# thu-ml/tianshou

Hardware: NVIDIA H100
Metric: transitions/sec through Algorithm.learn() (PPO, obs=17) (higher is better)
Workload: dtype f32 (MLP fwd/bwd, Adam), f64 (GAE scan, running return statistics)

## Files before the change

### include/ts_b200.h

```cpp
#ifndef TS_B200_H_
#define TS_B200_H_

#include <stddef.h>
#include <stdint.h>

#ifdef __cplusplus
extern "C" {
#endif

#define TS_B200_ABI_VERSION 1

typedef void* ts_stream_t;

enum { TS_F32 = 0, TS_F64 = 1 };

int ts_version(void);
const char* ts_last_error(void);
int64_t ts_launch_count(void);
void ts_reset_launch_count(void);

size_t ts_gae_workspace_bytes(int64_t n);
int ts_gae(const void* v_s, const void* v_s_next, int v_dtype, const double* rew,
           const uint8_t* terminated, const uint8_t* truncated, const uint8_t* extra_end,
           int terminated_ends, int64_t n, double gamma, double lam, double* rms_state,
// ... 47 lines not shown
                      ts_stream_t stream);
int ts_prio_update_weight(double* tree, int64_t bound, const int64_t* index, const void* td,
                          int td_dtype, int64_t n, double alpha, double eps, double* prio_minmax,
                          ts_stream_t stream);
int ts_prio_get_weight(const double* tree, int64_t bound, const int64_t* index, int64_t n,
                       const double* prio_minmax, double beta, int weight_norm, double* out,
                       ts_stream_t stream);

#define TS_AC_RELU 1
#define TS_AC_CATEGORICAL 2
typedef struct ts_actor_critic_desc {
    int32_t obs_dim;
    int32_t act_dim;
    int32_t hidden;
    int32_t flags;
    int64_t a_w1, a_b1, a_w2, a_b2, a_w3, a_b3, a_logstd;
    int64_t c_w1, c_b1, c_w2, c_b2, c_w3, c_b3;
    int64_t n_params;
} ts_actor_critic_desc;

int ts_critic_forward(const float* params, const ts_actor_critic_desc* desc ,
                      const float* obs0, float* v_out0, const float* obs1, float* v_out1,
                      int64_t n, ts_stream_t stream);
int ts_actor_logp(const float* params, const ts_actor_critic_desc* desc ,
                  const float* obs, const float* act, int64_t n, float* logp_out, float* mu_out,
                  ts_stream_t stream);

typedef struct ts_ppo_hparams {
    double eps_clip;
    double dual_clip;
    double vf_coef;
    double ent_coef;
    double max_grad_norm;
    double adv_eps;
    double lr, beta1, beta2, adam_eps, weight_decay;
    int32_t value_clip;
    int32_t advantage_normalization;
    int32_t loss_kind;
    int32_t optimizer;
} ts_ppo_hparams;
#define TS_LOSS_PPO 0
#define TS_LOSS_A2C 1
#define TS_OPT_ADAM 0
#define TS_OPT_RMSPROP 1

#define TS_PPO_STATS_STRIDE 8
// ... 7 lines not shown
                const float* logp_old, const float* v_s, const int32_t* perm, int64_t lo,
                int64_t hi, int64_t global_rows, const float* adv_moments, float* partials,
                int32_t* n_partials_out , ts_stream_t stream);
int ts_grad_reduce(const float* partials, int32_t n_partials, const ts_actor_critic_desc* desc,
                   float* grad, ts_stream_t stream);
int ts_minibatch_adv_sums(const float* adv, const int32_t* perm, int64_t lo, int64_t hi,
                          double* sums, ts_stream_t stream);
int ts_adv_moments_finalize(const double* sums, int64_t global_rows, float* out,
                            ts_stream_t stream);
int ts_clip_adam_step(float* params, float* grad, const float* partials, int32_t n_partials,
                      float* exp_avg, float* exp_avg_sq, int64_t* step_count,
                      const ts_actor_critic_desc* desc, const ts_ppo_hparams* hp, float* stats_row,
                      ts_stream_t stream);

int ts_ppo_update(float* params, float* grad, float* partials, float* exp_avg, float* exp_avg_sq,
                  int64_t* step_count, const ts_actor_critic_desc* desc, const ts_ppo_hparams* hp,
                  const float* obs, const float* obs_next, const float* act, const double* rew,
                  const uint8_t* terminated, const uint8_t* truncated, const uint8_t* extra_end,
                  float* v_s, float* returns, float* adv, const float* logp_old,
                  float* v_next_tmp, int64_t N, const int32_t* perm, int32_t repeat,
                  const int64_t* bounds , int32_t n_minibatch, int32_t recompute_adv,
                  double gamma, double lam, double* rms_state, double rms_eps, void* gae_ws,
                  void* adv_tmp, void* weight_image, float* stats, void* row_feed, ts_stream_t stream);

#define TS_PEER_HANDLE_BYTES 64
int ts_peer_alloc(int64_t bytes, void** ptr_out, uint8_t* handle_out );
int ts_peer_open(const uint8_t* handle, void** ptr_out);
int ts_peer_close(void* ptr);
int ts_peer_free(void* ptr);
int64_t ts_ppo_peer_buffer_bytes(const ts_actor_critic_desc* desc, int32_t world);

int ts_epoch_adv_sums(const float* adv, const int32_t* perm, int64_t lo0, int64_t mb_size, int64_t end,
                      int32_t n_minibatch, double* sums, ts_stream_t stream);
int ts_epoch_adv_finalize(const double* sums, int64_t lo0, int64_t mb_size, int64_t end, int32_t n_minibatch,
                          int32_t world, float* out, ts_stream_t stream);

int ts_ppo_epoch_multi(float* params, float* grad, float* partials, float* exp_avg, float* exp_avg_sq,
                       int64_t* step_count, const ts_actor_critic_desc* desc, const ts_ppo_hparams* hp,
                       const float* obs, const float* act, const float* adv, const float* returns,
                       const float* logp_old, const float* v_s, const int32_t* perm, int64_t lo0,
                       int64_t mb_size, int64_t end, int32_t n_minibatch, const float* adv_moments,
                       void* weight_image, float* stats, int32_t rank, int32_t world,
                       void* const* peer_buffers , ts_stream_t stream);

int ts_host_mt19937_permutation(uint32_t* key , int32_t* pos , int64_t n, int32_t* out);

// ... 139 lines not shown
```

### tianshou_b200/algorithm/modelfree/a2c.py

```python
from __future__ import annotations

import contextlib
import ctypes as C
import os
from abc import ABC
from dataclasses import dataclass
from typing import Any

import numpy as np
import torch

from ... import ops
from ..._cabi import GRAD_EXTRA, STATS_STRIDE, PPOHParams, load_library, to_device
from ...data import Batch, ReplayBuffer, SequenceSummaryStats
from ...parallel import world
from ...utils import RunningMeanStd
from ...utils.net.common import ActorCritic
from ..base import OnPolicyAlgorithm, TrainingStats
from ..flat_params import (
    DeviceScratch,
    FlatGroup,
    UnsupportedModelError,
    bind_optimizer,
    check_categorical_dist_fn,
    check_gaussian_dist_fn,
    optimizer_hyperparams,
)
# ... 15 lines not shown
def _upload(arr: np.ndarray, dev: torch.device, dtype: torch.dtype | None = None) -> torch.Tensor:
    t = to_device(arr, dev, non_blocking=True)
    if dtype is not None and t.dtype != dtype:
        t = t.to(dtype)
    return t


class ActorCriticOnPolicyAlgorithm(OnPolicyAlgorithm, ABC):

    minibatch_shuffle: str = "numpy"
    _shuffle_seed: int = 0
    _shuffle_epoch: int = 0

    def __init__(self, *, policy: ProbabilisticActorPolicy, critic: torch.nn.Module, optim: OptimizerFactory,
                 optim_include_actor: bool, max_grad_norm: float | None = None, gae_lambda: float = 0.95,
                 max_batchsize: int = 256, gamma: float = 0.99, return_scaling: bool = False,
                 rollout_partition: str = "per_rank", data_parallel: bool = True) -> None:
        super().__init__(policy=policy)
        if rollout_partition not in ("per_rank", "shared"):
            raise ValueError(f"rollout_partition must be 'per_rank' or 'shared', got {rollout_partition!r}")
        self.rollout_partition = rollout_partition
        self.data_parallel = bool(data_parallel)
        self._active_order: MinibatchOrder | None = None
        self.critic = critic
        assert 0.0 <= gae_lambda <= 1.0, f"GAE lambda should be in [0, 1] but got: {gae_lambda}"
        assert 0.0 <= gamma <= 1.0, f"discount factor gamma should be in [0, 1] but got: {gamma}"
        self.gae_lambda = gae_lambda
        self.max_batchsize = max_batchsize
        self._actor_critic = ActorCritic(self.policy.actor, self.critic)
        self._spec = parse_actor_critic(self.policy.actor, self.critic, split=not optim_include_actor)
        dev = next(self.policy.actor.parameters()).device
        if dev.type != "cuda":
            raise UnsupportedModelError(
                f"actor/critic live on {dev}; tianshou_b200 has no CPU path -- move them to a CUDA device first")
        if self._spec.categorical:
            check_categorical_dist_fn(self.policy.dist_fn, self._spec.act_dim, dev)
        else:
            check_gaussian_dist_fn(self.policy.dist_fn, self._spec.act_dim, dev)
        force_layered = os.environ.get("TS_B200_FORCE_LAYERED", "0") == "1"
        fused = fused_descriptor(self._spec) if optim_include_actor and not force_layered else None
        if fused is None:
            self._desc, self._layered = None, LayeredActorCritic(self._spec, dev)
            if self._ranks()[1] > 1:
                raise UnsupportedModelError("the layer-wise actor-critic path is single-GPU")
            self._flat = self._layered.critic_group
        else:
# ... 112 lines not shown
        batch.__dict__["info"] = Batch()
        batch.__dict__["policy"] = Batch()
        return batch, indices

    def _add_returns_and_advantages(self, batch: Batch, buffer: ReplayBuffer | None, indices: Any) -> Batch:
        self._flat.ensure_adopted()
        n = batch.obs.shape[0]
        v_s = self._buf("v_s", n, torch.float32)
        v_next = self._buf("v_next", n, torch.float32)
        r, w = self._ranks()
        if self._layered is not None:
            self._layered.critic_values(batch.obs, v_s)
            self._layered.critic_values(batch.obs_next, v_next)
        elif self.rollout_partition == "shared" and w > 1 and n % w == 0:
            import torch.distributed as dist
            lo, hi = r * (n // w), (r + 1) * (n // w)
            pair = self._buf("v_pair_local", (2, n // w), torch.float32)
            ops.critic_forward(self._flat.flat, self._desc, batch.obs[lo:hi], batch.obs_next[lo:hi], out=pair[0], out2=pair[1])
            full = self._buf("v_pair_full", (w, 2, n // w), torch.float32)
            dist.all_gather_into_tensor(full, pair)
            v_s.view(w, n // w).copy_(full[:, 0])
            v_next.view(w, n // w).copy_(full[:, 1])
        else:
            ops.critic_forward(self._flat.flat, self._desc, batch.obs, batch.obs_next, out=v_s, out2=v_next)
        rms = self._rms_device() if self.return_scaling else None
        adv = self._buf("adv", n, torch.float32)
        ret = self._buf("returns", n, torch.float32)
        moments = None
        if rms is not None and w > 1 and self.rollout_partition == "per_rank":
            moments = self._buf("rms_moments", 3, torch.float64)
        ops.gae(v_s, v_next, batch.rew, batch.terminated, batch.truncated, batch.get("_unfinished"),
                gamma=self.gamma, gae_lambda=self.gae_lambda, rms_state=rms, rms_eps=self._eps,
                out=(adv, ret), workspace=self._gae_workspace(n), batch_moments_out=moments)
        if moments is not None:
            self._merge_rms_across_ranks(rms, moments)
        batch.__dict__["v_s"], batch.__dict__["returns"], batch.__dict__["adv"] = v_s, ret, adv
        return batch

    def _gae_workspace(self, n: int) -> torch.Tensor:
        from ..._cabi import load_library
        need = int(load_library().ts_gae_workspace_bytes(n))
        return self._buf("gae_ws", max(need, 64), torch.uint8)

    def _rms_device(self) -> torch.Tensor:
        t = self._scratch.get("rms")
        if t is None:
            t = self._scratch["rms"] = self.ret_rms.device_state(self.device)
        return t

    def _rms_begin(self) -> None:
        if self.return_scaling:
            self._scratch["rms"] = self.ret_rms.device_state(self.device)

    def _rms_end(self) -> None:
        if self.return_scaling and "rms" in self._scratch:
            self.ret_rms.load_device_state(self._scratch.pop("rms"))

    def _merge_rms_across_ranks(self, rms: torch.Tensor, moments: torch.Tensor) -> None:
        from ...parallel import allgather_moments
        from ..._cabi import call, ptr, stream_ptr
        allm = allgather_moments(moments)
# ... 35 lines not shown
```

### tianshou_b200/algorithm/modelfree/ppo.py

```python
from __future__ import annotations

import ctypes as C
from typing import Any, Literal

import torch

from ... import ops
from ..._cabi import LOSS_A2C, call, ptr, stream_ptr
from ...data import Batch, ReplayBuffer
from ...data.batch import minibatch_bounds
from ...parallel import allreduce_sum_
from ..minibatch_order import shared_slice
from ..optim import OptimizerFactory
from .a2c import A2CTrainingStats, ActorCriticOnPolicyAlgorithm
from .reinforce import ProbabilisticActorPolicy


class FusedActorCriticUpdate(ActorCriticOnPolicyAlgorithm):

    recompute_adv: bool = False
    advantage_normalization: bool = False

    def _loss_hparams(self) -> Any:
        raise NotImplementedError
# ... 29 lines not shown
                        self._one_pass(batch, order.rows[r], bounds, hp, stats[r * n_mb:], r, rank, wsize)
            result = self._stats_from_device(stats)
        self._rms_end()
        self._flat.export_state(self.optim._optim)
        return result

    def _minibatch_adv_moments(self, batch: Batch, perm: torch.Tensor, lo: int, hi: int, world: int) -> torch.Tensor:
        st = stream_ptr(self.device)
        sums = self._buf("adv_sums", 2, torch.float64)
        call("ts_minibatch_adv_sums", ptr(batch.adv), ptr(perm), lo, hi, ptr(sums), st)
        if world > 1:
            allreduce_sum_(sums)
        adv_mom = self._buf("adv_mom", 2, torch.float32)
        call("ts_adv_moments_finalize", ptr(sums), (hi - lo) * world, ptr(adv_mom), st)
        return adv_mom

    def _device_passes(self, batch: Batch, perm_rows: torch.Tensor | None, bounds: list[tuple[int, int]], hp: Any,
                       stats: torch.Tensor, nrep: int, recompute: bool, feed: Any = None) -> None:
        f, dev = self._flat, self.device
        N, n_mb = batch.obs.shape[0], len(bounds)
        adv_tmp = self._buf("adv_tmp", 32 + 8 * n_mb, torch.uint8)
        adv_tmp.zero_()
        bounds_c = (C.c_int64 * (2 * n_mb))(*[x for b in bounds for x in b])
        call("ts_ppo_update", ptr(f.flat), ptr(f.grad), ptr(f.partials), ptr(f.exp_avg), ptr(f.exp_avg_sq), ptr(f.step_dev),
             C.byref(self._desc), C.byref(hp), ptr(batch.obs), ptr(batch.obs_next), ptr(batch.act),
             ptr(batch.rew), ptr(batch.terminated), ptr(batch.truncated), ptr(batch.get("_unfinished")),
             ptr(batch.v_s), ptr(batch.returns), ptr(batch.adv), ptr(batch.logp_old),
             ptr(self._buf("v_next", N, torch.float32)), N, ptr(perm_rows), nrep, bounds_c, n_mb,
             int(recompute), float(self.gamma), float(self.gae_lambda),
             ptr(self._rms_device()) if self.return_scaling else None, float(self._eps),
             ptr(self._gae_workspace(N)), ptr(adv_tmp), ptr(f.weight_image), ptr(stats), feed, stream_ptr(dev))

    def _peer_exchange(self, bounds: list[tuple[int, int]]):
        import os

        from ...parallel import PeerExchange
        if "peer_exchange" not in self._scratch:
            size = bounds[0][1] - bounds[0][0]
            regular = all(lo == bounds[0][0] + m * size and (m == len(bounds) - 1 or hi == lo + size)
                          for m, (lo, hi) in enumerate(bounds))
            usable = (os.environ.get("TS_B200_NO_P2P", "0") != "1" and regular
                      and self._flat.weight_image is not None and os.environ.get("TS_B200_FORCE_SIMT", "0") != "1")
            self._scratch["peer_exchange"] = PeerExchange.create(self._desc, self.device) if usable else None
        return self._scratch["peer_exchange"]

    def _fused_distributed_pass(self, batch: Batch, perm: torch.Tensor | None, bounds: list[tuple[int, int]], hp: Any,
                                stats: torch.Tensor, rank: int, wsize: int) -> None:
        f, st = self._flat, stream_ptr(self.device)
        ex = self._scratch["peer_exchange"]
        n_mb = len(bounds)
        lo0, size, end = bounds[0][0], bounds[0][1] - bounds[0][0], bounds[-1][1]
        adv_mom = None
        if self.advantage_normalization:
            sums = self._buf("epoch_adv_sums", 2 * n_mb, torch.float64)
# ... 120 lines not shown
```

### tianshou_b200/csrc/index.cu

```cuda
#include "common.cuh"

namespace {

using tsb::find_subbuffer;
using tsb::pymod;

struct BufMeta {
    const int64_t* offset;
    int64_t E;
    const uint8_t* done;
    const int64_t* last_index;
    const int64_t* lengths;
};

__device__ __forceinline__ int64_t next_one(const BufMeta& m, int64_t i) {
    const int64_t total = __ldg(m.offset + m.E);
    i = pymod(i, total);
    const int64_t e = find_subbuffer(m.offset, m.E, i);
    const int64_t start = __ldg(m.offset + e);
    int64_t len = __ldg(m.lengths + e);
    if (len < 1) len = 1;
    const int64_t last = __ldg(m.last_index + e);
    const int64_t end_flag = (m.done[i] != 0) | (i == last);
    return pymod(i - start + 1 - end_flag, len) + start;
// ... 181 lines not shown
    }
}
template <typename W>
__global__ void scatter_rows_kernel(const W* __restrict__ src, int64_t row_words,
                                    const int64_t* __restrict__ idx, int64_t n, W* __restrict__ dst) {
    const int64_t total = n * row_words;
    for (int64_t t = (int64_t)blockIdx.x * blockDim.x + threadIdx.x; t < total;
         t += (int64_t)gridDim.x * blockDim.x) {
        const int64_t p = t / row_words, w = t - p * row_words;
        dst[idx[p] * row_words + w] = src[t];
    }
}
__global__ void gather_bytes_kernel(const uint8_t* __restrict__ src, const int64_t* __restrict__ idx,
                                    int64_t n, uint8_t* __restrict__ dst) {
    const int64_t t = (int64_t)blockIdx.x * blockDim.x + threadIdx.x;
    if (t < n) dst[t] = src[idx[t]];
}

__global__ void narrow_kernel(const int64_t* __restrict__ src, int64_t n, int32_t* __restrict__ dst) {
    const int64_t t = (int64_t)blockIdx.x * blockDim.x + threadIdx.x;
    if (t < n) dst[t] = (int32_t)src[t];
}

inline unsigned blocks_for(int64_t n, int threads) { return (unsigned)((n + threads - 1) / threads); }

}

#define META_ARGS_OK(fn) \
    TS_REQUIRE(offset && done && last_index && lengths && E > 0, fn ": null buffer metadata")

extern "C" int ts_next_index(const int64_t* index, int64_t n, const int64_t* offset, int64_t E,
                             const uint8_t* done, const int64_t* last_index,
                             const int64_t* lengths, int64_t* out, ts_stream_t stream) {
    if (n == 0) return 0;
    META_ARGS_OK("ts_next_index");
    TS_REQUIRE(index && out, "ts_next_index: null index/out");
    BufMeta m{offset, E, done, last_index, lengths};
    step_index_kernel<true><<<blocks_for(n, 256), 256, 0, tsb::as_stream(stream)>>>(m, index, n, out);
    return tsb::check_launch("ts_next_index");
}

extern "C" int ts_prev_index(const int64_t* index, int64_t n, const int64_t* offset, int64_t E,
                             const uint8_t* done, const int64_t* last_index,
                             const int64_t* lengths, int64_t* out, ts_stream_t stream) {
    if (n == 0) return 0;
    META_ARGS_OK("ts_prev_index");
    TS_REQUIRE(index && out, "ts_prev_index: null index/out");
    BufMeta m{offset, E, done, last_index, lengths};
// ... 132 lines not shown
```

### tianshou_b200/csrc/mlp.cu

```cuda
#include <math.h>
#include <stdlib.h>

#include "common.cuh"
#include "optim_math.cuh"
#include "ppo_math.cuh"

namespace {

constexpr int H = 64;
constexpr int kRows = 128;
constexpr int kThreads = 256;
constexpr int LDH = H + 4;
constexpr int LDW3 = H + 4;
constexpr int LDO = 32;
constexpr int kMaxAct = 16;
constexpr int kMaxObs = 64;

struct NetOff {
    int w1t, b1, w2t, w2, b2, w3, b3, ls;
};
struct Layout {
    int KX, LDX, A;
    NetOff actor, critic;
    int X, H1, H2, ACT, DOUT, ROWV, RED;
// ... 648 lines not shown
int set_smem(K kernel, size_t bytes, const char* fn) {
    static thread_local size_t configured[tsb::kMaxDevices] = {};
    const int dev = tsb::device_ordinal();
    if (bytes > configured[dev]) {
        int optin = 0;
        TS_CUDA(cudaDeviceGetAttribute(&optin, cudaDevAttrMaxSharedMemoryPerBlockOptin, dev));
        TS_REQUIRE(bytes <= (size_t)optin, "%s: this network shape needs %zu bytes of shared memory per block, the device allows %d",
                   fn, bytes, optin);
        TS_CUDA(cudaFuncSetAttribute(kernel, cudaFuncAttributeMaxDynamicSharedMemorySize, (int)bytes));
        configured[dev] = bytes;
    }
    return 0;
}

}

namespace tsb {
bool tc_supported(const ts_actor_critic_desc& d);
int launch_ppo_grad_tc(const float* params, const ts_actor_critic_desc& d, const ts_ppo_hparams& hp, const float* obs,
                       const float* act, const float* adv, const float* ret, const float* logp_old, const float* v_s,
                       const int32_t* perm, int64_t lo, int64_t hi, int64_t global_rows, const float* adv_moments,
                       float* grad, cudaStream_t st);
int launch_forward_tc(int mode, const float* params, const ts_actor_critic_desc& d, const float* in0, float* out0,
                      const float* in1, float* out1, int64_t n, cudaStream_t st);
int launch_ppo_epoch_tc(float* params, const ts_actor_critic_desc& d, const ts_ppo_hparams& hp, const float* obs,
                        const float* act, const float* adv, const float* ret, const float* logp_old, const float* v_s,
                        const int32_t* perm, int64_t lo0, int64_t mb_size, int64_t end, int n_mb, const float* adv_moments,
                        float* partials, float* grad_scratch, float* exp_avg, float* exp_avg_sq, int64_t* step_count,
                        float* stats, void* weight_image, const PeerArgs& px, cudaStream_t st);
int64_t weight_image_bytes(const ts_actor_critic_desc& d);
static bool simt_forced() {
    static const bool f = [] { const char* e = getenv("TS_B200_FORCE_SIMT"); return e && e[0] == '1'; }();
    return f;
}
}

extern "C" int ts_critic_forward(const float* params, const ts_actor_critic_desc* desc,
                                 const float* obs0, float* v_out0, const float* obs1,
                                 float* v_out1, int64_t n, ts_stream_t stream) {
    if (check_desc(desc, "ts_critic_forward")) return 2;
    if (n == 0) return 0;
    TS_REQUIRE(params && obs0 && v_out0 && (!obs1 || v_out1), "ts_critic_forward: null pointer");
    if (tsb::tc_supported(*desc) && !tsb::simt_forced())
        return tsb::launch_forward_tc(0, params, *desc, obs0, v_out0, obs1, v_out1, n, tsb::as_stream(stream));
    const size_t smem = smem_bytes(*desc, 0);
    if (set_smem(critic_forward_kernel, smem, "ts_critic_forward")) return 1;
    const int64_t tiles = ((n + kRows - 1) / kRows) * (obs1 ? 2 : 1);
    const unsigned grid = (unsigned)tsb::imin((int64_t)tiles, tsb::num_sms());
    critic_forward_kernel<<<grid, kThreads, smem, tsb::as_stream(stream)>>>(params, *desc, obs0, v_out0, obs1, v_out1, n);
    return tsb::check_launch("ts_critic_forward");
}

extern "C" int ts_actor_logp(const float* params, const ts_actor_critic_desc* desc, const float* obs,
                             const float* act, int64_t n, float* logp_out, float* mu_out,
                             ts_stream_t stream) {
    if (check_desc(desc, "ts_actor_logp")) return 2;
    if (n == 0) return 0;
    TS_REQUIRE(params && obs && act && logp_out, "ts_actor_logp: null pointer");
    if (tsb::tc_supported(*desc) && !tsb::simt_forced())
        return tsb::launch_forward_tc(1, params, *desc, obs, logp_out, act, mu_out, n, tsb::as_stream(stream));
    const size_t smem = smem_bytes(*desc, 1);
    if (set_smem(actor_logp_kernel, smem, "ts_actor_logp")) return 1;
    const int64_t tiles = (n + kRows - 1) / kRows;
    const unsigned grid = (unsigned)tsb::imin((int64_t)tiles, tsb::num_sms());
    actor_logp_kernel<<<grid, kThreads, smem, tsb::as_stream(stream)>>>(params, *desc, obs, act, n, logp_out, mu_out);
    return tsb::check_launch("ts_actor_logp");
}

extern "C" int ts_ppo_grad(const float* params, const ts_actor_critic_desc* desc,
                           const ts_ppo_hparams* hp, const float* obs, const float* act,
                           const float* adv, const float* ret, const float* logp_old,
                           const float* v_s, const int32_t* perm, int64_t lo, int64_t hi,
                           int64_t global_rows, const float* adv_moments, float* partials,
                           int32_t* n_partials_out, ts_stream_t stream) {
    if (check_desc(desc, "ts_ppo_grad")) return 2;
    TS_REQUIRE(hp != nullptr, "ts_ppo_grad: null hparams");
    TS_REQUIRE(hi >= lo && global_rows > 0, "ts_ppo_grad: bad row range");
    if (n_partials_out) *n_partials_out = 0;
    if (hi == lo) return 0;
    TS_REQUIRE(params && obs && act && adv && ret && logp_old && v_s && partials && n_partials_out, "ts_ppo_grad: null pointer");
    {
        const int64_t tiles_ = (hi - lo + kRows - 1) / kRows;
        *n_partials_out = (int32_t)tsb::imin(tiles_, tsb::num_sms());
// ... 61 lines not shown
extern "C" int ts_make_permutation(uint64_t seed, int32_t first_epoch, int32_t n_epochs, int64_t n,
                                   int32_t* out, ts_stream_t stream) {
    if (n == 0 || n_epochs == 0) return 0;
    TS_REQUIRE(out && n > 0 && n < (1ll << 31) && n_epochs > 0, "ts_make_permutation: bad arguments");
    int bits = 1;
    while ((1ll << bits) < n) ++bits;
    const int half = (bits + 1) / 2 < 1 ? 1 : (bits + 1) / 2;
    const int64_t total = n * n_epochs;
    const unsigned grid = (unsigned)tsb::imin((int64_t)(total + 255) / 256, (int64_t)tsb::num_sms() * 8);
    permutation_kernel<<<grid, 256, 0, tsb::as_stream(stream)>>>(seed, first_epoch, n_epochs, n, half, out);
    return tsb::check_launch("ts_make_permutation");
}

extern "C" int ts_ppo_update(float* params, float* grad, float* partials, float* exp_avg, float* exp_avg_sq,
                             int64_t* step_count, const ts_actor_critic_desc* desc,
                             const ts_ppo_hparams* hp, const float* obs, const float* obs_next,
                             const float* act, const double* rew, const uint8_t* terminated,
                             const uint8_t* truncated, const uint8_t* extra_end, float* v_s,
                             float* returns, float* adv, const float* logp_old, float* v_next_tmp,
                             int64_t N, const int32_t* perm, int32_t repeat, const int64_t* bounds,
                             int32_t n_minibatch, int32_t recompute_adv, double gamma, double lam,
                             double* rms_state, double rms_eps, void* gae_ws, void* adv_tmp,
                             void* weight_image, float* stats, void* row_feed, ts_stream_t stream) {
    if (check_desc(desc, "ts_ppo_update")) return 2;
    TS_REQUIRE(hp && bounds && stats && partials && grad && repeat >= 0 && n_minibatch >= 0, "ts_ppo_update: bad arguments");
    TS_REQUIRE(!hp->advantage_normalization || adv_tmp, "ts_ppo_update: adv_tmp required");
    static const bool no_fuse = [] { const char* e = getenv("TS_B200_NO_FUSED_STEP"); return e && e[0] == '1'; }();
    const bool fused = tsb::tc_supported(*desc) && !tsb::simt_forced() && !no_fuse;
    double* adv_sums = static_cast<double*>(adv_tmp);
    float* adv_mom = adv_tmp ? reinterpret_cast<float*>(adv_sums + 2) : nullptr;
    float* epoch_mom = adv_tmp ? reinterpret_cast<float*>(static_cast<uint8_t*>(adv_tmp) + 32) : nullptr;
    bool regular = n_minibatch > 0;
    const int64_t lo0 = n_minibatch > 0 ? bounds[0] : 0, mb_size = n_minibatch > 0 ? bounds[1] - bounds[0] : 0;
    for (int m = 0; m < n_minibatch && regular; ++m) {
        regular = bounds[2 * m] == lo0 + (int64_t)m * mb_size && bounds[2 * m + 1] > bounds[2 * m] &&
                  (m == n_minibatch - 1 || bounds[2 * m + 1] == lo0 + (int64_t)(m + 1) * mb_size);
    }
    for (int r = 0; r < repeat; ++r) {
        if (recompute_adv && r > 0) {
            TS_REQUIRE(obs_next && rew && v_next_tmp && gae_ws, "ts_ppo_update: recompute needs obs_next/rew/scratch");
            if (int e = ts_critic_forward(params, desc, obs, v_s, obs_next, v_next_tmp, N, stream)) return e;
            if (int e = ts_gae(v_s, v_next_tmp, TS_F32, rew, terminated, truncated, extra_end, 1, N, gamma,
                               lam, rms_state, rms_eps, nullptr, adv, returns, TS_F32, gae_ws, stream)) return e;
        }
        const int32_t* pr = perm ? perm + (int64_t)r * N : nullptr;
        float* rows = stats + (int64_t)r * n_minibatch * TS_PPO_STATS_STRIDE;
        if (row_feed) {
            if (int e = ts_host_perm_feed_wait_row(row_feed, r, stream)) return e;
        }
        if (fused && regular) {
            const int64_t end = bounds[2 * n_minibatch - 1];
            if (hp->advantage_normalization) {
                epoch_adv_moments_kernel<<<n_minibatch, 1024, 0, tsb::as_stream(stream)>>>(adv, pr, lo0, mb_size, end, n_minibatch, epoch_mom);
                if (int e = tsb::check_launch("ts_ppo_update(adv moments)")) return e;
            }
            if (int e = tsb::launch_ppo_epoch_tc(params, *desc, *hp, obs, act, adv, returns, logp_old, v_s, pr, lo0, mb_size, end,
                                                 n_minibatch, hp->advantage_normalization ? epoch_mom : nullptr, partials, grad,
                                                 exp_avg, exp_avg_sq, step_count, rows, weight_image, tsb::PeerArgs{}, tsb::as_stream(stream))) return e;
            continue;
        }
        for (int m = 0; m < n_minibatch; ++m) {
            const int64_t lo = bounds[2 * m], hi = bounds[2 * m + 1];
            if (hp->advantage_normalization) {
                if (int e = ts_minibatch_adv_sums(adv, pr, lo, hi, adv_sums, stream)) return e;
// ... 60 lines not shown
```

### tianshou_b200/csrc/mlp_tc.cu

```cuda
#include <cuda_bf16.h>
#include <math.h>

#include <type_traits>

#include "common.cuh"
#include "optim_math.cuh"
#include "ppo_math.cuh"
#include "wgmma.cuh"

namespace {

constexpr int H = 64;
constexpr int kRows = 128;
constexpr int kThreads = 512;
constexpr int kCols = 16;
constexpr int kMaxAct = 16;
constexpr int NO = 16;

#ifdef TS_B200_DIAGNOSTICS
__device__ unsigned long long g_tc_timeline[32];
__device__ int g_tc_timeline_on = 0;
__device__ int g_tc_timeline_gate = 1;
__device__ __forceinline__ void tstamp(int slot) {
    if (g_tc_timeline_on && (int)blockIdx.x == g_tc_timeline_on - 1 && threadIdx.x == 0 && g_tc_timeline_gate) {
// ... 855 lines not shown
    SmemF s{};
    s.KXP = kxp;
    uint32_t o = 0;
    auto mat = [&](Mat& m, int rows, int cols) {
        m.base = sbase + o; m.part = mat_bytes(rows, cols); m.RS = (uint32_t)(cols / 8) * 128u; o += 3u * m.part;
    };
    mat(s.X, kRows, s.KXP);
    mat(s.H1, kRows, H);
    mat(s.W1, H, s.KXP);
    mat(s.W2, H, H);
    s.w3f = o;  o += kMaxAct * H * 4;
    s.b1 = o;   o += H * 4;
    s.b2 = o;   o += H * 4;
    s.b3 = o;   o += kMaxAct * 4;
    s.ls = o;   o += kMaxAct * 4;
    s.part = o; o += 2 * kRows * kMaxAct * 4;
    s.total = o;
    return s;
}

template <int MODE, int KXP>
__global__ void __launch_bounds__(kThreads, 1) forward_tc_kernel(
    const float* __restrict__ params, const ts_actor_critic_desc d, const float* __restrict__ in0,
    float* __restrict__ out0, const float* __restrict__ in1, float* __restrict__ out1, int64_t n) {
    extern __shared__ __align__(1024) uint8_t sm[];
    const int tid = threadIdx.x, lane = tid & 31;
    const uint32_t sbase = wg::smem_u32(sm);
    uint8_t* sm0 = sm - sbase;
    const SmemF S = make_smem_f(KXP, sbase);
    const int out_dim = MODE == 0 ? 1 : d.act_dim;
    const NetG g = MODE == 0 ? NetG{d.c_w1, d.c_b1, d.c_w2, d.c_b2, d.c_w3, d.c_b3, -1}
                             : NetG{d.a_w1, d.a_b1, d.a_w2, d.a_b2, d.a_w3, d.a_b3, d.a_logstd};
    stage_chunks(sm0, S.W1, H, d.obs_dim, S.KXP, [&](int o) { return params + g.w1 + (int64_t)o * d.obs_dim; });
    stage_chunks(sm0, S.W2, H, H, H, [&](int o) { return params + g.w2 + (int64_t)o * H; });
    float* w3f = reinterpret_cast<float*>(sm + S.w3f);
    float* b1 = reinterpret_cast<float*>(sm + S.b1);
    float* b2 = reinterpret_cast<float*>(sm + S.b2);
    float* b3 = reinterpret_cast<float*>(sm + S.b3);
    float* ls = reinterpret_cast<float*>(sm + S.ls);
    float* part = reinterpret_cast<float*>(sm + S.part);
    for (int e = tid; e < kMaxAct * H; e += kThreads) w3f[e] = (e >> 6) < out_dim ? __ldg(params + g.w3 + e) : 0.0f;
    for (int e = tid; e < H; e += kThreads) { b1[e] = __ldg(params + g.b1 + e); b2[e] = __ldg(params + g.b2 + e); }
    if (tid < kMaxAct) {
        b3[tid] = tid < out_dim ? __ldg(params + g.b3 + tid) : 0.0f;
        ls[tid] = (MODE == 1 && tid < out_dim) ? expf(__ldg(params + g.ls + tid)) : 1.0f;
    }

    const int64_t tiles_per = (n + kRows - 1) / kRows;
    const int64_t tiles = tiles_per * ((MODE == 0 && in1) ? 2 : 1);
    const int64_t my_n = tiles > (int64_t)blockIdx.x ? (tiles - blockIdx.x + gridDim.x - 1) / gridDim.x : 0;
    auto tile_of = [&](int64_t k) { return (int64_t)blockIdx.x + k * gridDim.x; };
    auto tile_src = [&](int64_t t, const float*& src, int64_t& row0, int& nrows, bool& second) {
        second = t >= tiles_per;
        row0 = (second ? t - tiles_per : t) * kRows;
        nrows = (int)tsb::imin((int64_t)kRows, n - row0);
        src = (MODE == 0 && second) ? in1 : in0;
    };
    auto x_load = [&](int64_t k, float (&xv)[8]) {
        const float* src; int64_t row0; int nrows; bool second;
        tile_src(tile_of(k), src, row0, nrows, second);
        chunk_load(kRows, d.obs_dim, S.KXP, [&](int r) {
            return r < nrows ? src + (row0 + r) * d.obs_dim : (const float*)nullptr;
        }, xv);
    };
    const int half = tid >> 8;
    const int r0 = lay_row0() + wg::frag_row(0);

    float xv[8];
    if (my_n > 0) x_load(0, xv);
    for (int64_t k = 0; k < my_n; ++k) {
        const float* src; int64_t row0; int nrows; bool second;
        tile_src(tile_of(k), src, row0, nrows, second);
        __syncthreads();
        chunk_store(sm0, S.X, kRows, S.KXP, xv);
        if (k + 1 < my_n) x_load(k + 1, xv);
        publish();
        float acc[kCols], h[kCols];
        if (S.KXP == 16) wg_gemm<2 * kCols, 1, 0, 0>(acc, S.X, lay_row0(), S.W1, lay_col0());
        else wg_gemm<2 * kCols, 2, 0, 0>(acc, S.X, lay_row0(), S.W1, lay_col0());
        epi_tanh(sm0, S.H1, acc, b1);
        publish();
        wg_gemm<2 * kCols, H / 16, 0, 0>(acc, S.H1, lay_row0(), S.W2, lay_col0());
#pragma unroll
        for (int e = 0; e < kCols; ++e) h[e] = tanh_mufu(acc[e] + b2[lay_col0() + wg::frag_col(e)]);
        for (int a = 0; a < out_dim; ++a) {
            float p0 = 0.0f, p1 = 0.0f;
#pragma unroll
            for (int i = 0; i < kCols / 4; ++i) {
                const float2 w = *reinterpret_cast<const float2*>(w3f + a * H + lay_col0() + wg::frag_col(4 * i));
                p0 = fmaf(h[4 * i], w.x, p0); p0 = fmaf(h[4 * i + 1], w.y, p0);
                p1 = fmaf(h[4 * i + 2], w.x, p1); p1 = fmaf(h[4 * i + 3], w.y, p1);
            }
            p0 += __shfl_xor_sync(0xffffffffu, p0, 1); p0 += __shfl_xor_sync(0xffffffffu, p0, 2);
            p1 += __shfl_xor_sync(0xffffffffu, p1, 1); p1 += __shfl_xor_sync(0xffffffffu, p1, 2);
            if ((lane & 3) == 0) {
                part[(half * kMaxAct + a) * kRows + r0] = p0;
                part[(half * kMaxAct + a) * kRows + r0 + 8] = p1;
            }
        }
        __syncthreads();
        if (tid < nrows) {
            const int r = tid;
            if (MODE == 0) {
                (second ? out1 : out0)[row0 + r] = (part[r] + part[kMaxAct * kRows + r]) + b3[0];
            } else {
                float lp = 0.0f;
                for (int a = 0; a < out_dim; ++a) {
                    const float mu = (part[a * kRows + r] + part[(kMaxAct + a) * kRows + r]) + b3[a];
                    lp += ppo::normal_logp_term(__ldg(in1 + (row0 + r) * out_dim + a), mu, ls[a]);
                    if (out1) out1[(row0 + r) * out_dim + a] = mu;
                }
                out0[row0 + r] = lp;
            }
        }
    }
}

}

#ifdef TS_B200_DIAGNOSTICS
extern "C" int ts_tc_timeline(int32_t enable, uint64_t* out32 ) {
    int on = enable;
    TS_CUDA(cudaMemcpyToSymbol(g_tc_timeline_on, &on, sizeof(int)));
    if (out32) TS_CUDA(cudaMemcpyFromSymbol(out32, g_tc_timeline, 32 * sizeof(unsigned long long)));
    return 0;
}
#endif
// ... 54 lines not shown
        cfg.gridDim = dim3(grid); cfg.blockDim = dim3(kThreads); cfg.dynamicSmemBytes = S.total; cfg.stream = st;
        cudaLaunchAttribute attr[1];
        attr[0].id = cudaLaunchAttributeCooperative;
        attr[0].val.cooperative = 1;
        cfg.attrs = attr; cfg.numAttrs = 1;
        const int64_t zero = 0;
        uint8_t* wimg = weight_image ? static_cast<uint8_t*>(weight_image) + kCtlBytes : nullptr;
        if (wimg) {
            TS_CUDA(cudaMemsetAsync(wimg, 0, 2 * (size_t)S.wblk_bytes, st));
            weight_image_build_kernel<KXP><<<(unsigned)((d.n_params + 255) / 256), 256, 0, st>>>(params, d, wimg);
            if (int e = check_launch("ts_ppo_update(weight image)")) return e;
        }
        TS_CUDA(cudaLaunchKernelEx(&cfg, ppo_tc_kernel<true, KXP>, (const float*)params, d, hp, obs, act, adv, ret, logp_old, v_s,
                                   perm, lo0, mb_size, end, n_mb, zero, adv_moments, partials, opt, wimg, px));
        return check_launch("ts_ppo_epoch(tc)");
    });
}

int64_t weight_image_bytes(const ts_actor_critic_desc& d) {
    return tc_supported(d) ? (int64_t)kCtlBytes + 2 * (int64_t)make_smem(kxp_of(d.obs_dim), 0).wblk_bytes : 0;
}

int launch_forward_tc(int mode, const float* params, const ts_actor_critic_desc& d, const float* in0, float* out0,
                      const float* in1, float* out1, int64_t n, cudaStream_t st) {
    return with_kxp(d.obs_dim, [&](auto kxp) {
        constexpr int KXP = decltype(kxp)::value;
        constexpr size_t smem = make_smem_f(KXP, 0).total;
        const int64_t tiles = ((n + kRows - 1) / kRows) * ((mode == 0 && in1) ? 2 : 1);
        const unsigned grid = (unsigned)imin(tiles, num_sms());
        if (mode == 0) {
            if (int e = opt_in_smem<forward_tc_kernel<0, KXP>>(smem)) return e;
            forward_tc_kernel<0, KXP><<<grid, kThreads, smem, st>>>(params, d, in0, out0, in1, out1, n);
        } else {
            if (int e = opt_in_smem<forward_tc_kernel<1, KXP>>(smem)) return e;
            forward_tc_kernel<1, KXP><<<grid, kThreads, smem, st>>>(params, d, in0, out0, in1, out1, n);
        }
        return check_launch(mode == 0 ? "ts_critic_forward(tc)" : "ts_actor_logp(tc)");
    });
}
}
```

### tianshou_b200/ops.py

```python
from __future__ import annotations

import ctypes as C
from dataclasses import dataclass

import numpy as np
import torch

from . import _cabi
from ._cabi import TS_F32, TS_F64, ActorCriticDesc, PPOHParams, call, ptr, stream_ptr, to_device


def _dev(device: torch.device | str | None) -> torch.device:
    _cabi.require_cuda()
    if device is None:
        return torch.device("cuda", torch.cuda.current_device())
    d = torch.device(device)
    if d.type != "cuda":
        raise _cabi.ExtensionMissingError(f"tianshou_b200 kernels need a CUDA device, got {d}")
    return d


def _dt(t: torch.dtype) -> int:
    if t == torch.float32:
        return TS_F32
# ... 213 lines not shown
         stream_ptr(tree.device))
    return out


def segtree_sample(tree: torch.Tensor, bound: int, u: torch.Tensor) -> torch.Tensor:
    out = torch.empty(u.numel(), dtype=torch.int64, device=tree.device)
    call("ts_segtree_sample", ptr(tree), bound, ptr(u), u.numel(), ptr(out), stream_ptr(tree.device))
    return out


def critic_forward(params: torch.Tensor, desc: ActorCriticDesc, obs: torch.Tensor,
                   obs2: torch.Tensor | None = None,
                   out: torch.Tensor | None = None, out2: torch.Tensor | None = None):
    n = obs.shape[0]
    if out is None:
        out = torch.empty(n, dtype=torch.float32, device=obs.device)
    if obs2 is not None and out2 is None:
        out2 = torch.empty(n, dtype=torch.float32, device=obs.device)
    call("ts_critic_forward", ptr(params), C.byref(desc), ptr(obs), ptr(out), ptr(obs2), ptr(out2), n,
         stream_ptr(obs.device))
    return (out, out2) if obs2 is not None else out


def actor_logp(params: torch.Tensor, desc: ActorCriticDesc, obs: torch.Tensor, act: torch.Tensor,
               want_mu: bool = False, out: torch.Tensor | None = None):
    n = obs.shape[0]
    if out is None:
        out = torch.empty(n, dtype=torch.float32, device=obs.device)
    mu = torch.empty((n, desc.act_dim), dtype=torch.float32, device=obs.device) if want_mu else None
    call("ts_actor_logp", ptr(params), C.byref(desc), ptr(obs), ptr(act), n, ptr(out), ptr(mu),
         stream_ptr(obs.device))
    return (out, mu) if want_mu else out


def make_permutation(seed: int, first_epoch: int, n_epochs: int, n: int, device: torch.device) -> torch.Tensor:
    out = torch.empty((n_epochs, n), dtype=torch.int32, device=device)
    call("ts_make_permutation", C.c_uint64(seed & (2**64 - 1)), int(first_epoch), int(n_epochs), int(n),
         ptr(out), stream_ptr(device))
    return out


def narrow_i64_i32(src: torch.Tensor) -> torch.Tensor:
    out = torch.empty(src.shape, dtype=torch.int32, device=src.device)
    call("ts_narrow_i64_i32", ptr(src), src.numel(), ptr(out), stream_ptr(src.device))
    return out

# ... 3 lines not shown
```

Before: 26.71 million.

## Deduplicate critic forward on obs_next rows that alias the following obs row

Adds a mark/compact kernel pair that detects rows where obs_next[i] is bitwise equal to obs[i+1] and builds a compacted list of the non-aliased rows. The tensor-core critic forward then evaluates only obs plus those extra rows and scatters V(obs[i+1]) into v_next[i], roughly halving critic forward work for contiguous rollouts. The map is built once per batch and reused when the PPO update recomputes advantages across repeats. In exchange it adds two small kernels, indexed gathers and scatters, and a device-side row count that the kernel must read.

Measured after the change: 28.07 million (median of 6 runs). 5.1% higher.

```diff
diff --git a/include/ts_b200.h b/include/ts_b200.h
--- a/include/ts_b200.h
+++ b/include/ts_b200.h
@@ -93,6 +93,12 @@
 int ts_critic_forward(const float* params, const ts_actor_critic_desc* desc ,
                       const float* obs0, float* v_out0, const float* obs1, float* v_out1,
                       int64_t n, ts_stream_t stream);
+int64_t ts_next_alias_workspace_bytes(int64_t n);
+int ts_next_alias_map(const float* obs, const float* obs_next, int64_t n, int32_t obs_dim, uint8_t* alias,
+                      int32_t* extra, int32_t* n_extra, void* workspace, ts_stream_t stream);
+int ts_critic_forward_dedup(const float* params, const ts_actor_critic_desc* desc , const float* obs,
+                            const float* obs_next, const uint8_t* alias, const int32_t* extra,
+                            const int32_t* n_extra, float* v_s, float* v_next, int64_t n, ts_stream_t stream);
 int ts_actor_logp(const float* params, const ts_actor_critic_desc* desc ,
                   const float* obs, const float* act, int64_t n, float* logp_out, float* mu_out,
                   ts_stream_t stream);
@@ -146,6 +152,17 @@
                   const int64_t* bounds , int32_t n_minibatch, int32_t recompute_adv,
                   double gamma, double lam, double* rms_state, double rms_eps, void* gae_ws,
                   void* adv_tmp, void* weight_image, float* stats, void* row_feed, ts_stream_t stream);
+int ts_ppo_update_dedup(float* params, float* grad, float* partials, float* exp_avg, float* exp_avg_sq,
+                        int64_t* step_count, const ts_actor_critic_desc* desc, const ts_ppo_hparams* hp,
+                        const float* obs, const float* obs_next, const float* act, const double* rew,
+                        const uint8_t* terminated, const uint8_t* truncated, const uint8_t* extra_end,
+                        float* v_s, float* returns, float* adv, const float* logp_old,
+                        float* v_next_tmp, int64_t N, const int32_t* perm, int32_t repeat,
+                        const int64_t* bounds , int32_t n_minibatch, int32_t recompute_adv,
+                        double gamma, double lam, double* rms_state, double rms_eps, void* gae_ws,
+                        void* adv_tmp, void* weight_image, float* stats, void* row_feed,
+                        const uint8_t* next_alias, const int32_t* next_extra, const int32_t* n_next_extra,
+                        ts_stream_t stream);
 
 #define TS_PEER_HANDLE_BYTES 64
 int ts_peer_alloc(int64_t bytes, void** ptr_out, uint8_t* handle_out );
diff --git a/tianshou_b200/algorithm/modelfree/a2c.py b/tianshou_b200/algorithm/modelfree/a2c.py
--- a/tianshou_b200/algorithm/modelfree/a2c.py
+++ b/tianshou_b200/algorithm/modelfree/a2c.py
@@ -3,6 +3,7 @@
 import contextlib
 import ctypes as C
 import os
+import weakref
 from abc import ABC
 from dataclasses import dataclass
 from typing import Any
@@ -64,6 +65,7 @@
         self.rollout_partition = rollout_partition
         self.data_parallel = bool(data_parallel)
         self._active_order: MinibatchOrder | None = None
+        self._next_alias: tuple[Any, Any, ops.NextAliasMap] | None = None
         self.critic = critic
         assert 0.0 <= gae_lambda <= 1.0, f"GAE lambda should be in [0, 1] but got: {gae_lambda}"
         assert 0.0 <= gamma <= 1.0, f"discount factor gamma should be in [0, 1] but got: {gamma}"
@@ -222,7 +224,11 @@
             v_s.view(w, n // w).copy_(full[:, 0])
             v_next.view(w, n // w).copy_(full[:, 1])
         else:
-            ops.critic_forward(self._flat.flat, self._desc, batch.obs, batch.obs_next, out=v_s, out2=v_next)
+            amap = self._next_alias_map(batch, build=buffer is not None)
+            if amap is not None:
+                ops.critic_forward_dedup(self._flat.flat, self._desc, batch.obs, batch.obs_next, amap, out=v_s, out2=v_next)
+            else:
+                ops.critic_forward(self._flat.flat, self._desc, batch.obs, batch.obs_next, out=v_s, out2=v_next)
         rms = self._rms_device() if self.return_scaling else None
         adv = self._buf("adv", n, torch.float32)
         ret = self._buf("returns", n, torch.float32)
@@ -237,6 +243,20 @@
         batch.__dict__["v_s"], batch.__dict__["returns"], batch.__dict__["adv"] = v_s, ret, adv
         return batch
 
+    def _next_alias_map(self, batch: Batch, build: bool = False) -> ops.NextAliasMap | None:
+        obs, obs_next = batch.obs, batch.obs_next
+        if build:
+            n = obs.shape[0]
+            amap = ops.NextAliasMap(self._buf("next_alias", n, torch.uint8), self._buf("next_extra", n, torch.int32),
+                                    self._buf("next_extra_count", 1, torch.int32))
+            need = int(load_library().ts_next_alias_workspace_bytes(n))
+            ops.next_alias_map(obs, obs_next, out=amap, workspace=self._buf("next_alias_ws", max(need, 4), torch.uint8))
+            self._next_alias = (weakref.ref(obs), weakref.ref(obs_next), amap)
+        if self._next_alias is None:
+            return None
+        ref_obs, ref_next, amap = self._next_alias
+        return amap if ref_obs() is obs and ref_next() is obs_next else None
+
     def _gae_workspace(self, n: int) -> torch.Tensor:
         from ..._cabi import load_library
         need = int(load_library().ts_gae_workspace_bytes(n))
diff --git a/tianshou_b200/algorithm/modelfree/ppo.py b/tianshou_b200/algorithm/modelfree/ppo.py
--- a/tianshou_b200/algorithm/modelfree/ppo.py
+++ b/tianshou_b200/algorithm/modelfree/ppo.py
@@ -75,14 +75,16 @@
         adv_tmp = self._buf("adv_tmp", 32 + 8 * n_mb, torch.uint8)
         adv_tmp.zero_()
         bounds_c = (C.c_int64 * (2 * n_mb))(*[x for b in bounds for x in b])
-        call("ts_ppo_update", ptr(f.flat), ptr(f.grad), ptr(f.partials), ptr(f.exp_avg), ptr(f.exp_avg_sq), ptr(f.step_dev),
+        amap = self._next_alias_map(batch) if recompute else None
+        call("ts_ppo_update_dedup", ptr(f.flat), ptr(f.grad), ptr(f.partials), ptr(f.exp_avg), ptr(f.exp_avg_sq), ptr(f.step_dev),
              C.byref(self._desc), C.byref(hp), ptr(batch.obs), ptr(batch.obs_next), ptr(batch.act),
              ptr(batch.rew), ptr(batch.terminated), ptr(batch.truncated), ptr(batch.get("_unfinished")),
              ptr(batch.v_s), ptr(batch.returns), ptr(batch.adv), ptr(batch.logp_old),
              ptr(self._buf("v_next", N, torch.float32)), N, ptr(perm_rows), nrep, bounds_c, n_mb,
              int(recompute), float(self.gamma), float(self.gae_lambda),
              ptr(self._rms_device()) if self.return_scaling else None, float(self._eps),
-             ptr(self._gae_workspace(N)), ptr(adv_tmp), ptr(f.weight_image), ptr(stats), feed, stream_ptr(dev))
+             ptr(self._gae_workspace(N)), ptr(adv_tmp), ptr(f.weight_image), ptr(stats), feed,
+             *((ptr(amap.alias), ptr(amap.extra), ptr(amap.count)) if amap is not None else (None, None, None)), stream_ptr(dev))
 
     def _peer_exchange(self, bounds: list[tuple[int, int]]):
         import os
diff --git a/tianshou_b200/csrc/index.cu b/tianshou_b200/csrc/index.cu
--- a/tianshou_b200/csrc/index.cu
+++ b/tianshou_b200/csrc/index.cu
@@ -227,8 +227,87 @@
     if (t < n) dst[t] = (int32_t)src[t];
 }
 
+constexpr int kAliasThreads = 256;
+
+__global__ void __launch_bounds__(kAliasThreads) next_alias_mark_kernel(
+    const uint32_t* __restrict__ obs, const uint32_t* __restrict__ obs_next, int64_t n, int width,
+    uint8_t* __restrict__ alias, int32_t* __restrict__ block_extra) {
+    const int lane = threadIdx.x & 31;
+    const int64_t i0 = (int64_t)blockIdx.x * kAliasThreads + (threadIdx.x & ~31);
+    const int64_t rows = tsb::imin(32, n - 1 - i0);
+    const uint32_t* a = obs_next + i0 * width;
+    const uint32_t* b = obs + (i0 + 1) * width;
+    unsigned differs = 0u;
+    for (int64_t w = lane; w < rows * width; w += 32) {
+        if (a[w] != b[w]) differs |= 1u << (unsigned)(w / width);
+    }
+    differs = __reduce_or_sync(0xffffffffu, differs);
+    const int64_t i = i0 + lane;
+    const bool same = lane < rows && !((differs >> lane) & 1u);
+    if (i < n) alias[i] = same ? 1 : 0;
+    const int cnt = __syncthreads_count(i < n && !same);
+    if (threadIdx.x == 0) block_extra[blockIdx.x] = cnt;
+}
+
+__global__ void __launch_bounds__(kAliasThreads) next_alias_compact_kernel(
+    const uint8_t* __restrict__ alias, int64_t n, const int32_t* __restrict__ block_extra,
+    int32_t* __restrict__ extra, int32_t* __restrict__ n_extra) {
+    __shared__ int s_warp[kAliasThreads / 32];
+    __shared__ int s_base;
+    const int tid = threadIdx.x, lane = tid & 31, warp = tid >> 5;
+    int before_blocks = 0;
+    for (int b = tid; b < (int)blockIdx.x; b += kAliasThreads) before_blocks += block_extra[b];
+#pragma unroll
+    for (int off = 16; off > 0; off >>= 1) before_blocks += __shfl_xor_sync(0xffffffffu, before_blocks, off);
+    if (lane == 0) s_warp[warp] = before_blocks;
+    __syncthreads();
+    if (tid == 0) {
+        int base = 0;
+        for (int w = 0; w < kAliasThreads / 32; ++w) base += s_warp[w];
+        s_base = base;
+    }
+    __syncthreads();
+    const int64_t i = (int64_t)blockIdx.x * kAliasThreads + tid;
+    const bool keep = i < n && alias[i] == 0;
+    const unsigned bal = __ballot_sync(0xffffffffu, keep);
+    const int base = s_base;
+    __syncthreads();
+    if (lane == 0) s_warp[warp] = __popc(bal);
+    __syncthreads();
+    int before = 0, total = 0;
+    for (int w = 0; w < kAliasThreads / 32; ++w) {
+        if (w < warp) before += s_warp[w];
+        total += s_warp[w];
+    }
+    if (keep) extra[base + before + __popc(bal & ((1u << lane) - 1u))] = (int32_t)i;
+    if (blockIdx.x == gridDim.x - 1 && tid == 0) *n_extra = base + total;
+}
+
 inline unsigned blocks_for(int64_t n, int threads) { return (unsigned)((n + threads - 1) / threads); }
 
+}
+
+extern "C" int64_t ts_next_alias_workspace_bytes(int64_t n) {
+    return n > 0 ? 4 * (int64_t)blocks_for(n, kAliasThreads) : 0;
+}
+
+extern "C" int ts_next_alias_map(const float* obs, const float* obs_next, int64_t n, int32_t obs_dim, uint8_t* alias,
+                                 int32_t* extra, int32_t* n_extra, void* workspace, ts_stream_t stream) {
+    TS_REQUIRE(n >= 0 && n < (1ll << 31) && obs_dim >= 1, "ts_next_alias_map: bad shape");
+    TS_REQUIRE(n_extra, "ts_next_alias_map: null n_extra");
+    cudaStream_t st = tsb::as_stream(stream);
+    if (n == 0) {
+        TS_CUDA(cudaMemsetAsync(n_extra, 0, sizeof(int32_t), st));
+        return 0;
+    }
+    TS_REQUIRE(obs && obs_next && alias && extra && workspace, "ts_next_alias_map: null pointer");
+    int32_t* block_extra = static_cast<int32_t*>(workspace);
+    const unsigned grid = blocks_for(n, kAliasThreads);
+    next_alias_mark_kernel<<<grid, kAliasThreads, 0, st>>>(reinterpret_cast<const uint32_t*>(obs),
+                                                           reinterpret_cast<const uint32_t*>(obs_next), n, obs_dim, alias, block_extra);
+    if (tsb::check_launch("ts_next_alias_map/mark")) return 1;
+    next_alias_compact_kernel<<<grid, kAliasThreads, 0, st>>>(alias, n, block_extra, extra, n_extra);
+    return tsb::check_launch("ts_next_alias_map");
 }
 
 #define META_ARGS_OK(fn) \
diff --git a/tianshou_b200/csrc/mlp.cu b/tianshou_b200/csrc/mlp.cu
--- a/tianshou_b200/csrc/mlp.cu
+++ b/tianshou_b200/csrc/mlp.cu
@@ -694,7 +694,8 @@
                        const int32_t* perm, int64_t lo, int64_t hi, int64_t global_rows, const float* adv_moments,
                        float* grad, cudaStream_t st);
 int launch_forward_tc(int mode, const float* params, const ts_actor_critic_desc& d, const float* in0, float* out0,
-                      const float* in1, float* out1, int64_t n, cudaStream_t st);
+                      const float* in1, float* out1, int64_t n, const uint8_t* alias, const int32_t* extra,
+                      const int32_t* n_extra, cudaStream_t st);
 int launch_ppo_epoch_tc(float* params, const ts_actor_critic_desc& d, const ts_ppo_hparams& hp, const float* obs,
                         const float* act, const float* adv, const float* ret, const float* logp_old, const float* v_s,
                         const int32_t* perm, int64_t lo0, int64_t mb_size, int64_t end, int n_mb, const float* adv_moments,
@@ -714,13 +715,24 @@
     if (n == 0) return 0;
     TS_REQUIRE(params && obs0 && v_out0 && (!obs1 || v_out1), "ts_critic_forward: null pointer");
     if (tsb::tc_supported(*desc) && !tsb::simt_forced())
-        return tsb::launch_forward_tc(0, params, *desc, obs0, v_out0, obs1, v_out1, n, tsb::as_stream(stream));
+        return tsb::launch_forward_tc(0, params, *desc, obs0, v_out0, obs1, v_out1, n, nullptr, nullptr, nullptr, tsb::as_stream(stream));
     const size_t smem = smem_bytes(*desc, 0);
     if (set_smem(critic_forward_kernel, smem, "ts_critic_forward")) return 1;
     const int64_t tiles = ((n + kRows - 1) / kRows) * (obs1 ? 2 : 1);
     const unsigned grid = (unsigned)tsb::imin((int64_t)tiles, tsb::num_sms());
     critic_forward_kernel<<<grid, kThreads, smem, tsb::as_stream(stream)>>>(params, *desc, obs0, v_out0, obs1, v_out1, n);
     return tsb::check_launch("ts_critic_forward");
+}
+
+extern "C" int ts_critic_forward_dedup(const float* params, const ts_actor_critic_desc* desc, const float* obs,
+                                       const float* obs_next, const uint8_t* alias, const int32_t* extra,
+                                       const int32_t* n_extra, float* v_s, float* v_next, int64_t n, ts_stream_t stream) {
+    if (check_desc(desc, "ts_critic_forward_dedup")) return 2;
+    if (n == 0) return 0;
+    TS_REQUIRE(params && obs && obs_next && alias && extra && n_extra && v_s && v_next, "ts_critic_forward_dedup: null pointer");
+    if (tsb::tc_supported(*desc) && !tsb::simt_forced())
+        return tsb::launch_forward_tc(0, params, *desc, obs, v_s, obs_next, v_next, n, alias, extra, n_extra, tsb::as_stream(stream));
+    return ts_critic_forward(params, desc, obs, v_s, obs_next, v_next, n, stream);
 }
 
 extern "C" int ts_actor_logp(const float* params, const ts_actor_critic_desc* desc, const float* obs,
@@ -730,7 +742,7 @@
     if (n == 0) return 0;
     TS_REQUIRE(params && obs && act && logp_out, "ts_actor_logp: null pointer");
     if (tsb::tc_supported(*desc) && !tsb::simt_forced())
-        return tsb::launch_forward_tc(1, params, *desc, obs, logp_out, act, mu_out, n, tsb::as_stream(stream));
+        return tsb::launch_forward_tc(1, params, *desc, obs, logp_out, act, mu_out, n, nullptr, nullptr, nullptr, tsb::as_stream(stream));
     const size_t smem = smem_bytes(*desc, 1);
     if (set_smem(actor_logp_kernel, smem, "ts_actor_logp")) return 1;
     const int64_t tiles = (n + kRows - 1) / kRows;
@@ -838,8 +850,27 @@
                              int32_t n_minibatch, int32_t recompute_adv, double gamma, double lam,
                              double* rms_state, double rms_eps, void* gae_ws, void* adv_tmp,
                              void* weight_image, float* stats, void* row_feed, ts_stream_t stream) {
+    return ts_ppo_update_dedup(params, grad, partials, exp_avg, exp_avg_sq, step_count, desc, hp, obs, obs_next, act, rew,
+                               terminated, truncated, extra_end, v_s, returns, adv, logp_old, v_next_tmp, N, perm, repeat,
+                               bounds, n_minibatch, recompute_adv, gamma, lam, rms_state, rms_eps, gae_ws, adv_tmp,
+                               weight_image, stats, row_feed, nullptr, nullptr, nullptr, stream);
+}
+
+extern "C" int ts_ppo_update_dedup(float* params, float* grad, float* partials, float* exp_avg, float* exp_avg_sq,
+                                   int64_t* step_count, const ts_actor_critic_desc* desc,
+                                   const ts_ppo_hparams* hp, const float* obs, const float* obs_next,
+                                   const float* act, const double* rew, const uint8_t* terminated,
+                                   const uint8_t* truncated, const uint8_t* extra_end, float* v_s,
+                                   float* returns, float* adv, const float* logp_old, float* v_next_tmp,
+                                   int64_t N, const int32_t* perm, int32_t repeat, const int64_t* bounds,
+                                   int32_t n_minibatch, int32_t recompute_adv, double gamma, double lam,
+                                   double* rms_state, double rms_eps, void* gae_ws, void* adv_tmp,
+                                   void* weight_image, float* stats, void* row_feed, const uint8_t* next_alias,
+                                   const int32_t* next_extra, const int32_t* n_next_extra, ts_stream_t stream) {
     if (check_desc(desc, "ts_ppo_update")) return 2;
     TS_REQUIRE(hp && bounds && stats && partials && grad && repeat >= 0 && n_minibatch >= 0, "ts_ppo_update: bad arguments");
+    TS_REQUIRE((next_alias != nullptr) == (next_extra != nullptr) && (next_alias != nullptr) == (n_next_extra != nullptr),
+               "ts_ppo_update: the next-observation alias map is three pointers, all or none");
     TS_REQUIRE(!hp->advantage_normalization || adv_tmp, "ts_ppo_update: adv_tmp required");
     static const bool no_fuse = [] { const char* e = getenv("TS_B200_NO_FUSED_STEP"); return e && e[0] == '1'; }();
     const bool fused = tsb::tc_supported(*desc) && !tsb::simt_forced() && !no_fuse;
@@ -855,7 +886,9 @@
     for (int r = 0; r < repeat; ++r) {
         if (recompute_adv && r > 0) {
             TS_REQUIRE(obs_next && rew && v_next_tmp && gae_ws, "ts_ppo_update: recompute needs obs_next/rew/scratch");
-            if (int e = ts_critic_forward(params, desc, obs, v_s, obs_next, v_next_tmp, N, stream)) return e;
+            if (int e = next_alias ? ts_critic_forward_dedup(params, desc, obs, obs_next, next_alias, next_extra, n_next_extra,
+                                                             v_s, v_next_tmp, N, stream)
+                                   : ts_critic_forward(params, desc, obs, v_s, obs_next, v_next_tmp, N, stream)) return e;
             if (int e = ts_gae(v_s, v_next_tmp, TS_F32, rew, terminated, truncated, extra_end, 1, N, gamma,
                                lam, rms_state, rms_eps, nullptr, adv, returns, TS_F32, gae_ws, stream)) return e;
         }
diff --git a/tianshou_b200/csrc/mlp_tc.cu b/tianshou_b200/csrc/mlp_tc.cu
--- a/tianshou_b200/csrc/mlp_tc.cu
+++ b/tianshou_b200/csrc/mlp_tc.cu
@@ -901,7 +901,8 @@
 template <int MODE, int KXP>
 __global__ void __launch_bounds__(kThreads, 1) forward_tc_kernel(
     const float* __restrict__ params, const ts_actor_critic_desc d, const float* __restrict__ in0,
-    float* __restrict__ out0, const float* __restrict__ in1, float* __restrict__ out1, int64_t n) {
+    float* __restrict__ out0, const float* __restrict__ in1, float* __restrict__ out1, int64_t n,
+    const uint8_t* __restrict__ alias , const int32_t* __restrict__ extra, const int32_t* __restrict__ n_extra) {
     extern __shared__ __align__(1024) uint8_t sm[];
     const int tid = threadIdx.x, lane = tid & 31;
     const uint32_t sbase = wg::smem_u32(sm);
@@ -925,21 +926,25 @@
         ls[tid] = (MODE == 1 && tid < out_dim) ? expf(__ldg(params + g.ls + tid)) : 1.0f;
     }
 
+    const bool dedup = MODE == 0 && alias != nullptr;
     const int64_t tiles_per = (n + kRows - 1) / kRows;
-    const int64_t tiles = tiles_per * ((MODE == 0 && in1) ? 2 : 1);
+    const int64_t n2 = (MODE == 0 && in1) ? (dedup ? (int64_t)__ldg(n_extra) : n) : 0;
+    const int64_t tiles = tiles_per + (n2 + kRows - 1) / kRows;
     const int64_t my_n = tiles > (int64_t)blockIdx.x ? (tiles - blockIdx.x + gridDim.x - 1) / gridDim.x : 0;
     auto tile_of = [&](int64_t k) { return (int64_t)blockIdx.x + k * gridDim.x; };
     auto tile_src = [&](int64_t t, const float*& src, int64_t& row0, int& nrows, bool& second) {
         second = t >= tiles_per;
         row0 = (second ? t - tiles_per : t) * kRows;
-        nrows = (int)tsb::imin((int64_t)kRows, n - row0);
+        nrows = (int)tsb::imin((int64_t)kRows, (second ? n2 : n) - row0);
         src = (MODE == 0 && second) ? in1 : in0;
     };
     auto x_load = [&](int64_t k, float (&xv)[8]) {
         const float* src; int64_t row0; int nrows; bool second;
         tile_src(tile_of(k), src, row0, nrows, second);
         chunk_load(kRows, d.obs_dim, S.KXP, [&](int r) {
-            return r < nrows ? src + (row0 + r) * d.obs_dim : (const float*)nullptr;
+            if (r >= nrows) return (const float*)nullptr;
+            const int64_t row = (dedup && second) ? (int64_t)__ldg(extra + row0 + r) : row0 + r;
+            return src + row * d.obs_dim;
         }, xv);
     };
     const int half = tid >> 8;
@@ -981,7 +986,14 @@
         if (tid < nrows) {
             const int r = tid;
             if (MODE == 0) {
-                (second ? out1 : out0)[row0 + r] = (part[r] + part[kMaxAct * kRows + r]) + b3[0];
+                const float v = (part[r] + part[kMaxAct * kRows + r]) + b3[0];
+                const int64_t row = row0 + r;
+                if (!second) {
+                    out0[row] = v;
+                    if (dedup && row > 0 && __ldg(alias + row - 1)) out1[row - 1] = v;
+                } else {
+                    out1[dedup ? (int64_t)__ldg(extra + row) : row] = v;
+                }
             } else {
                 float lp = 0.0f;
                 for (int a = 0; a < out_dim; ++a) {
@@ -1082,18 +1094,19 @@
 }
 
 int launch_forward_tc(int mode, const float* params, const ts_actor_critic_desc& d, const float* in0, float* out0,
-                      const float* in1, float* out1, int64_t n, cudaStream_t st) {
+                      const float* in1, float* out1, int64_t n, const uint8_t* alias, const int32_t* extra,
+                      const int32_t* n_extra, cudaStream_t st) {
     return with_kxp(d.obs_dim, [&](auto kxp) {
         constexpr int KXP = decltype(kxp)::value;
         constexpr size_t smem = make_smem_f(KXP, 0).total;
-        const int64_t tiles = ((n + kRows - 1) / kRows) * ((mode == 0 && in1) ? 2 : 1);
+        const int64_t tiles = ((n + kRows - 1) / kRows) * ((mode == 0 && in1 && !alias) ? 2 : 1);
         const unsigned grid = (unsigned)imin(tiles, num_sms());
         if (mode == 0) {
             if (int e = opt_in_smem<forward_tc_kernel<0, KXP>>(smem)) return e;
-            forward_tc_kernel<0, KXP><<<grid, kThreads, smem, st>>>(params, d, in0, out0, in1, out1, n);
+            forward_tc_kernel<0, KXP><<<grid, kThreads, smem, st>>>(params, d, in0, out0, in1, out1, n, alias, extra, n_extra);
         } else {
             if (int e = opt_in_smem<forward_tc_kernel<1, KXP>>(smem)) return e;
-            forward_tc_kernel<1, KXP><<<grid, kThreads, smem, st>>>(params, d, in0, out0, in1, out1, n);
+            forward_tc_kernel<1, KXP><<<grid, kThreads, smem, st>>>(params, d, in0, out0, in1, out1, n, nullptr, nullptr, nullptr);
         }
         return check_launch(mode == 0 ? "ts_critic_forward(tc)" : "ts_actor_logp(tc)");
     });
diff --git a/tianshou_b200/ops.py b/tianshou_b200/ops.py
--- a/tianshou_b200/ops.py
+++ b/tianshou_b200/ops.py
@@ -259,6 +259,41 @@
     return (out, out2) if obs2 is not None else out
 
 
+@dataclass
+class NextAliasMap:
+
+    alias: torch.Tensor
+    extra: torch.Tensor
+    count: torch.Tensor
+
+
+def next_alias_map(obs: torch.Tensor, obs_next: torch.Tensor, out: NextAliasMap | None = None,
+                   workspace: torch.Tensor | None = None) -> NextAliasMap:
+    n, dev = obs.shape[0], obs.device
+    assert obs.dtype == torch.float32 and obs_next.dtype == torch.float32 and obs.shape == obs_next.shape
+    if out is None:
+        out = NextAliasMap(torch.empty(n, dtype=torch.uint8, device=dev), torch.empty(n, dtype=torch.int32, device=dev),
+                           torch.empty(1, dtype=torch.int32, device=dev))
+    need = int(_cabi.load_library().ts_next_alias_workspace_bytes(n))
+    if workspace is None or workspace.numel() < need:
+        workspace = torch.empty(max(need, 4), dtype=torch.uint8, device=dev)
+    call("ts_next_alias_map", ptr(obs), ptr(obs_next), n, obs[0].numel() if n else 1, ptr(out.alias), ptr(out.extra),
+         ptr(out.count), ptr(workspace), stream_ptr(dev))
+    return out
+
+
+def critic_forward_dedup(params: torch.Tensor, desc: ActorCriticDesc, obs: torch.Tensor, obs_next: torch.Tensor,
+                         amap: NextAliasMap, out: torch.Tensor | None = None, out2: torch.Tensor | None = None):
+    n = obs.shape[0]
+    if out is None:
+        out = torch.empty(n, dtype=torch.float32, device=obs.device)
+    if out2 is None:
+        out2 = torch.empty(n, dtype=torch.float32, device=obs.device)
+    call("ts_critic_forward_dedup", ptr(params), C.byref(desc), ptr(obs), ptr(obs_next), ptr(amap.alias), ptr(amap.extra),
+         ptr(amap.count), ptr(out), ptr(out2), n, stream_ptr(obs.device))
+    return out, out2
+
+
 def actor_logp(params: torch.Tensor, desc: ActorCriticDesc, obs: torch.Tensor, act: torch.Tensor,
                want_mu: bool = False, out: torch.Tensor | None = None):
     n = obs.shape[0]
```
